# YukunXia/SuperPoint-Stereo-Visual-Odometry

Measured on AMD Instinct MI355X. Metric: stereo frames/sec (1241x376 KITTI), higher is better.
Workload: dtype f32

## Files before the change

### superpoint-stereo-visual-odometry_amd/csrc/conv_wino2.hip.h

```cpp
#pragma once
#include <hip/hip_runtime.h>
#include <stdint.h>
#include <type_traits>
#include <vector>
#include "conv_mfma.hip.h"

#ifndef SPVO_STATIC_BANDS
#define SPVO_STATIC_BANDS 1
#endif

namespace spvo {

#ifndef WINO_STORE_AUX
#define WINO_STORE_AUX 0
#endif

struct WinoTile {
  static constexpr int CK = 8, TH = 8, TW = 32, LW = TW + 8, LH = TH + 2;
  static constexpr int IN_FLOATS = CK * LH * LW;
  static constexpr int U_FLOATS = 16 * CK * CO_TILE;
  static constexpr int W_FLOATS = U_FLOATS + CO_TILE;
  static constexpr int V_FLOATS = 16 * CK * 64;
  static constexpr int RAW_OFF = 0, U_OFF = 2 * IN_FLOATS, V_OFF = U_OFF + 2 * W_FLOATS;
  static constexpr int LDS_BYTES = (V_OFF + 2 * V_FLOATS) * 4;
};

constexpr int WINO2_LDS_BYTES = WinoTile::LDS_BYTES + 16;

inline std::vector<float> pack_conv_weights_wino2(const float *w, const float *bias, int cout, int cin, int cot = CO_TILE) {
  constexpr int CK = WinoTile::CK;
  const int co_tiles = (cout + cot - 1) / cot, nch = cin / CK, ncq = cot / 16;
  const int u_floats = 16 * CK * cot, w_floats = u_floats + cot;
  std::vector<float> out((size_t)co_tiles * nch * w_floats, 0.f);
  static const double G[4][3] = {{1, 0, 0}, {0.5, 0.5, 0.5}, {0.5, -0.5, 0.5}, {0, 0, 1}};
  for (int ct = 0; ct < co_tiles; ++ct)
    for (int ch = 0; ch < nch; ++ch) {
      float *slab = out.data() + ((size_t)ct * nch + ch) * w_floats;
      for (int o = 0; o < cot; ++o) {
        const int co = ct * cot + o;
        if (co >= cout) continue;
        for (int c = 0; c < CK; ++c) {
          const float *g = w + ((size_t)co * cin + ch * CK + c) * 9;
          double t[4][3];
          for (int a = 0; a < 4; ++a)
            for (int k = 0; k < 3; ++k) t[a][k] = G[a][0] * g[0 * 3 + k] + G[a][1] * g[1 * 3 + k] + G[a][2] * g[2 * 3 + k];
          const int lane = 16 * (c & 3) + (o & 15), s = c >> 2, cq = o >> 4;
          for (int a = 0; a < 4; ++a)
            for (int b = 0; b < 4; ++b)
              slab[((((a * 4 + b) >> 1) * ncq + cq) * 64 + lane) * 4 + 2 * ((a * 4 + b) & 1) + s] = (float)(t[a][0] * G[b][0] + t[a][1] * G[b][1] + t[a][2] * G[b][2]);
        }
        if (ch == 0) slab[u_floats + o] = bias[co];
      }
    }
  return out;
}

template <bool POOL, bool RELU, int TAG = 0, bool ODD = false, bool NARROW = false>
__global__ __launch_bounds__(512, 2) void conv_wino2_kernel(const ConvArgs a) {
  using T = WinoTile;
  constexpr int CK = T::CK, LW = T::LW, LH = T::LH, LW4 = LW / 4;
  constexpr int COT = NARROW ? 32 : 64, NCQ = COT / 16, NBLK = NARROW ? 1 : 2;
  constexpr int U_FL = 16 * CK * COT, W_FL = U_FL + COT;
  constexpr int IN_V4 = T::IN_FLOATS / 4, W_V4 = W_FL / 4;
  constexpr int NIT_R = (IN_V4 + 511) / 512, NIT_U = (W_V4 + 511) / 512;
  typedef float f32x2 __attribute__((ext_vector_type(2)));
  typedef float f32x4v __attribute__((ext_vector_type(4)));

  extern __shared__ __attribute__((aligned(16))) float smem[];

  const int tid = threadIdx.x;
  const int lane = tid & 63;
  const int c16 = lane & 15, g4 = lane >> 4;
  const int wave = __builtin_amdgcn_readfirstlane(tid >> 6);
  const int cq = wave % NCQ, tb = wave / NCQ;
  const size_t in_plane = (size_t)a.in_hp * a.in_wp;
  const size_t out_plane = (size_t)a.out_hp * a.out_wp;
  const int n_tiles = a.tiles_x * a.tiles_y * a.co_tiles * a.batch;

  struct TileRef { const float *in_base, *w_base; int x0, y0, ct, img; };
  auto decode = [&](int id) {
    TileRef t;
    const int tx = id % a.tiles_x;
    id /= a.tiles_x;
    const int ty = id % a.tiles_y;
    id /= a.tiles_y;
    t.ct = id % a.co_tiles;
    t.img = id / a.co_tiles;
    t.x0 = tx * T::TW;
    t.y0 = ty * T::TH;
    t.in_base = a.in + ((size_t)t.img * a.in_ctot + a.in_coff) * in_plane + (size_t)(t.y0 + PADY - 1) * a.in_wp + (t.x0 + PADX - 4);
    t.w_base = a.wpack + (size_t)t.ct * a.n_chunks * W_FL;
    return t;
  };

  unsigned roff[NIT_R];
#pragma unroll
  for (int it = 0; it < NIT_R; ++it) {
    const int idx = min(it * 512 + tid, IN_V4 - 1);
    const int ci = idx / (LH * LW4);
    const int rem = idx - ci * (LH * LW4);
    const int r = rem / LW4;
    const int q = rem - r * LW4;
    roff[it] = 4u * (unsigned)(ci * (int)in_plane + r * a.in_wp + q * 4);
  }
  auto issue_raw = [&](const TileRef &t, int chunk, float *buf) {
    const char *inb = reinterpret_cast<const char *>(t.in_base + (size_t)chunk * CK * in_plane);
#pragma unroll
    for (int it = 0; it < NIT_R; ++it)
      if (it < NIT_R - 1 || it * 512 + tid < IN_V4) glds16(reinterpret_cast<const float *>(inb + roff[it]), buf + (it * 512 + wave * 64) * 4);
  };
// ... 106 lines not shown
      if (q.id < n_tiles) q.t = decode(q.id);
    }
  };
  Cursor cu{cur, 0, tile_id};
  issue_raw(cu.t, 0, smem + T::RAW_OFF);
  issue_u(cu.t, 0, smem + T::U_OFF);
  advance(cu);
  if (cu.id < n_tiles) issue_raw(cu.t, cu.chunk, smem + T::RAW_OFF + T::IN_FLOATS);
  Cursor cr = cu;
  advance(cr);
  asm volatile("s_waitcnt vmcnt(0)\n\ts_barrier" ::: "memory");
  transform(smem + T::RAW_OFF, smem + T::V_OFF);

#ifdef WINO_STAMPS
  unsigned long long st_dma = 0, st_bar = 0, st_mfma = 0, st_epi = 0, st_items = 0;
  const unsigned long long st_t0 = __builtin_amdgcn_s_memtime(), st_r0 = __builtin_amdgcn_s_memrealtime();
#endif
  int k = 0;
  bool drained = true;
  constexpr unsigned OOB = 0xFFFFFFFFu;

  while (tile_id < n_tiles) {
    if (a.sched) {
      if (tid == 0) dyn_fetch = band_lo(band) + band_wgs(band) + atomicAdd(a.sched + band, 1);
    } else {
      nxt_id = tile_id + gridDim.x;
    }

    f32x4v acc[16][NBLK];
    auto item = [&](auto first_tag, bool publish) {
      constexpr bool FIRST = decltype(first_tag)::value;
#ifdef WINO_STAMPS
      const unsigned long long ts0 = __builtin_amdgcn_s_memtime();
#endif
      if (!drained) asm volatile("s_waitcnt vmcnt(0)" ::: "memory");
      drained = false;
#ifdef WINO_STAMPS
      const unsigned long long ts1 = __builtin_amdgcn_s_memtime();
#endif
      if (publish && tid == 0) *sched_slot = dyn_fetch < band_hi(band) ? dyn_fetch : n_tiles;
      asm volatile("s_waitcnt lgkmcnt(0)\n\ts_barrier" ::: "memory");
      if (publish) nxt_id = __builtin_amdgcn_readfirstlane(*sched_slot);
#ifdef WINO_STAMPS
      const unsigned long long ts2 = __builtin_amdgcn_s_memtime();
      st_dma += ts1 - ts0; st_bar += ts2 - ts1;
#endif
      const float *ub = smem + T::U_OFF + (k & 1) * T::W_FLOATS;
      const float *vb = smem + T::V_OFF + (k & 1) * T::V_FLOATS;
      float *u_next = smem + T::U_OFF + ((k + 1) & 1) * T::W_FLOATS;
      float *raw_next2 = smem + T::RAW_OFF + (k & 1) * T::IN_FLOATS;
      const float *raw_next = smem + T::RAW_OFF + ((k + 1) & 1) * T::IN_FLOATS;
      float *v_next = smem + T::V_OFF + ((k + 1) & 1) * T::V_FLOATS;
      const f32x4v *vb4 = reinterpret_cast<const f32x4v *>(vb);
      {
        f32x4v avq[2];
        f32x4v bv[4];
        const f32x4v *ub4 = reinterpret_cast<const f32x4v *>(ub);
        auto lda = [&](int g, int p) { avq[p] = ub4[a_lane + (2 * g + p) * (64 * NCQ)]; };
        auto ld = [&](int g, int x) {
          if constexpr (NARROW) {
            const f32x2 b2 = reinterpret_cast<const f32x2 *>(vb)[b_lane + (4 * g + x) * 256];
            bv[x][0] = b2[0]; bv[x][1] = b2[1];
          } else {
            bv[x] = vb4[b_lane + (4 * g + x) * 128];
          }
        };
        lda(0, 0); lda(0, 1);
#pragma unroll
        for (int x = 0; x < 4; ++x) ld(0, x);
#pragma unroll
        for (int g = 0; g < 4; ++g) {
          constexpr int QN = NARROW ? 8 : 16;
#pragma unroll
          for (int q = 0; q < QN; ++q) {
            const int s = NARROW ? q >> 2 : q >> 3, x = NARROW ? q & 3 : (q >> 1) & 3, blk = NARROW ? 0 : q & 1;
            const float a_op = avq[x >> 1][2 * (x & 1) + s];
            if (FIRST && s == 0) acc[4 * g + x][blk] = __builtin_amdgcn_mfma_f32_16x16x4f32(a_op, bv[x][2 * blk + s], f32x4v{0.f, 0.f, 0.f, 0.f}, 0, 0, 0);
            else acc[4 * g + x][blk] = __builtin_amdgcn_mfma_f32_16x16x4f32(a_op, bv[x][2 * blk + s], acc[4 * g + x][blk], 0, 0, 0);
            __builtin_amdgcn_sched_barrier(0);
#ifndef WINO2_ABL
#define WINO2_ABL 0
#endif
#ifndef WINO2_SPREAD
#define WINO2_SPREAD 0
#endif
            const int slot = QN * g + q;
            if (!(WINO2_ABL & 2)) {
              if (WINO2_SPREAD) {
                if (slot >= 1 && slot < 1 + 2 * NIT_U && (slot & 1) && cu.id < n_tiles) issue_u_piece(cu.t, cu.chunk, u_next, (slot - 1) >> 1);
                if (slot >= 1 + 2 * NIT_U && slot < 1 + 2 * NIT_U + 2 * NIT_R && (slot & 1) && cr.id < n_tiles) issue_raw_piece(cr.t, cr.chunk, raw_next2, (slot - 1 - 2 * NIT_U) >> 1);
              } else {
                if (slot == 1 && cu.id < n_tiles) issue_u(cu.t, cu.chunk, u_next);
                if (slot == 5 && cr.id < n_tiles) issue_raw(cr.t, cr.chunk, raw_next2);
              }
            }
            if (!(WINO2_ABL & 4) && g < 3 && q >= QN - 4) {
              ld(g + 1, q - (QN - 4));
              if (q == QN - 4 + (NARROW ? 1 : 0)) lda(g + 1, 0);
              if (q == QN - 1) lda(g + 1, 1);
            }
            if constexpr (NARROW) {
              if (!(WINO2_ABL & 1) && slot >= 8 && slot < 28) xf_step(raw_next, v_next, slot - 8);
            } else {
              if (!(WINO2_ABL & 1) && slot >= 16 && slot < 56 && !(slot & 1)) xf_step(raw_next, v_next, (slot - 16) >> 1);
            }
            __builtin_amdgcn_sched_barrier(0);
          }
        }
      }
      if (FIRST) {
        const float bias_a = g4 ? 0.f : ub[U_FL + cq * 16 + c16];
#pragma unroll
        for (int blk = 0; blk < NBLK; ++blk) acc[5][blk] = __builtin_amdgcn_mfma_f32_16x16x4f32(bias_a, 1.0f, acc[5][blk], 0, 0, 0);
      }
      advance(cu);
      advance(cr);
      ++k;
#ifdef WINO_STAMPS
      st_mfma += __builtin_amdgcn_s_memtime() - ts2;
      ++st_items;
#endif
    };
    item(std::true_type{}, false);
    for (int c = 1; c < a.n_chunks; ++c) item(std::false_type{}, a.sched != nullptr && c == 1);

    asm volatile("s_waitcnt vmcnt(0)" ::: "memory");
    drained = true;

#ifdef WINO_STAMPS
    const unsigned long long te0 = __builtin_amdgcn_s_memtime();
#endif
    float *co_base = a.out + (((size_t)cur.img * a.out_ctot + a.out_coff) + (size_t)cur.ct * COT + cq * 16) * out_plane;
    const __amdgpu_buffer_rsrc_t rsrc = __builtin_amdgcn_make_buffer_rsrc(co_base, 0, 0x7FFFFFFF, 0x00020000);
    const int oplane = (int)out_plane;
    const int kmax = a.cout - (cur.ct * COT + cq * 16 + 4 * g4);
    auto relu = [](float v) { return RELU ? __builtin_amdgcn_fmed3f(v, 0.f, __builtin_inff()) : v; };
#pragma unroll
    for (int blk = 0; blk < NBLK; ++blk) {
// ... 60 lines not shown
```

### superpoint-stereo-visual-odometry_amd/csrc/spvo_core.hip

```cpp
#include "spvo_internal.hip.h"
#include <mutex>
#include "conv_mfma.hip.h"
#include "conv_f16.hip.h"
#include "conv_bf16x3.hip.h"
#include "conv_wino2.hip.h"
#include "conv_wino4.hip.h"
#include "heads.hip.h"
#include "conv_i8.hip.h"
#include "conv_i8_fused.hip.h"
#include "heads_i8.hip.h"

namespace spvo_int {

thread_local std::string g_error;
HostDiag g_diag;

int fail(spvo_ctx *c, int code, const char *fmt, ...) {
  char buf[512];
  va_list ap;
  va_start(ap, fmt);
  vsnprintf(buf, sizeof buf, fmt, ap);
  va_end(ap);
  if (c) c->error = buf;
  g_error = buf;
  return code;
}

int stage_id(spvo_ctx *c, const std::string &name) {
  for (size_t i = 0; i < c->stages.size(); ++i)
    if (c->stages[i].name == name) return (int)i;
  Stage s;
  s.name = name;
  c->stages.push_back(s);
  return (int)c->stages.size() - 1;
}

namespace {
const char *const kTuningNames[] = {"winograd", "wino4", "wino4_item", "wino_narrow", "wino_dynamic", "winograd_min_tiles", "wino4_min_tiles", "merge_siblings", "heads_fused",
                                    "heads_on_net", "heads_split", "match_fused", "fp32_split", "prematch", "spin_wait", "trunk_timing", "solve_timing", "nms_first", "upload_side", "inject_launch_failure", "int8_fused", "pair_always", "preprocess_fused", "heads_keep_raw", "tail_streams", "solve_collect_first", "graphs", "solve_fuse", "solve_keep", "sift_describe_form", "sift_pair_waves_per_cu", "conv_variant"};
constexpr int kTuningCount = sizeof kTuningNames / sizeof kTuningNames[0];
std::mutex g_tuning_mutex;
bool g_tuning_set[kTuningCount] = {};
int g_tuning_value[kTuningCount] = {};
int tuning_index(const char *name) {
  for (int i = 0; name && i < kTuningCount; ++i)
    if (std::strcmp(name, kTuningNames[i]) == 0) return i;
  return -1;
}
}
int tuning(const char *name, int dflt) {
  const int i = tuning_index(name);
  if (i < 0) return dflt;
  std::lock_guard<std::mutex> lock(g_tuning_mutex);
  return g_tuning_set[i] ? g_tuning_value[i] : dflt;
}

bool spin_wait_enabled() { return tuning("spin_wait", 0) != 0; }
hipError_t wait_event(hipEvent_t ev) {
  if (spin_wait_enabled()) {
    for (long spins = 0; spins < 20000000; ++spins) {
      const hipError_t e = hipEventQuery(ev);
      if (e != hipErrorNotReady) return e;
      __builtin_ia32_pause();
    }
  }
  return hipEventSynchronize(ev);
}

hipEvent_t get_event(spvo_ctx *c) {
  if (!c->free_events.empty()) {
    hipEvent_t e = c->free_events.back();
    c->free_events.pop_back();
    return e;
  }
  hipEvent_t e;
  (void)hipEventCreate(&e);
  return e;
}

void resolve_pending(spvo_ctx *c) {
  if (c->pending.empty()) return;
  for (auto &p : c->pending) {
    float ms = 0;
    (void)hipEventSynchronize(p.e1);
    if (hipEventElapsedTime(&ms, p.e0, p.e1) == hipSuccess) {
      c->stages[p.stage].total_ms += ms;
      c->stages[p.stage].calls += 1;
      c->stages[p.stage].flops_sum += p.flops;
      c->stages[p.stage].bytes_sum += p.bytes;
    }
    c->free_events.push_back(p.e0);
// ... 694 lines not shown
          HIP_TRY(c, hipMemcpy(op.d_b, b, (size_t)op.cout * 4, hipMemcpyHostToDevice));
          continue;
        }
        const int ckg = op.ks == 3 ? 1 : 2;
        if (op.cin % (8 * ckg) || op.in_c_off % 8) return fail(c, SPVO_ERR_IO, "op %u: cin %d / channel offset %d do not fit the split-fp32 chunking (%d)", i, op.cin, op.in_c_off, 8 * ckg);
        op.ck = 8 * ckg;
        op.n_chunks = op.cin / op.ck;
        op.co_tiles = (op.cout + CO_TILE - 1) / CO_TILE;
        int ck_unused;
        choose_variant(op.ks, ti.H, ti.W, op.co_tiles, c->cfg.max_batch, pool, c->num_cus, &op.wr, &op.wc, &ck_unused, true);
        const std::vector<unsigned short> pk = pack_conv_weights_s3(w, b, op.cout, op.cin, op.ks, ckg);
        int rc = dev_alloc(c, &op.d_ws3, pk.size(), false);
        if (rc) return rc;
        HIP_TRY(c, hipMemcpy(op.d_ws3, pk.data(), pk.size() * sizeof(unsigned short), hipMemcpyHostToDevice));
        continue;
      }
      if (op.cin == 1) {
        if (pool || add) return fail(c, SPVO_ERR_IO, "op %u: single-channel-input layers have no pooling / residual form", i);
        int rc = dev_alloc(c, &op.d_w, (size_t)op.cout * taps, false);
        if (rc) return rc;
        if ((rc = dev_alloc(c, &op.d_b, op.cout, false))) return rc;
        HIP_TRY(c, hipMemcpy(op.d_w, w, (size_t)op.cout * taps * 4, hipMemcpyHostToDevice));
        HIP_TRY(c, hipMemcpy(op.d_b, b, (size_t)op.cout * 4, hipMemcpyHostToDevice));
        continue;
      }
      op.co_tiles = (op.cout + CO_TILE - 1) / CO_TILE;
      choose_variant(op.ks, ti.H, ti.W, op.co_tiles, c->cfg.max_batch, pool, c->num_cus, &op.wr, &op.wc, &op.ck);
      {
        const bool wino_on = tuning("winograd", 1) != 0;
        const long wtiles = (long)((ti.W + WinoTile::TW - 1) / WinoTile::TW) * ((ti.H + WinoTile::TH - 1) / WinoTile::TH) * op.co_tiles * c->cfg.max_batch;
        const long min_tiles = tuning("winograd_min_tiles", 3 * c->num_cus / 4);
        const bool eligible = wino_on && op.ks == 3 && !bn && !add && (op.cin % WinoTile::CK) == 0 && (!pool || ((ti.H % 2) == 0 && (ti.W % 2) == 0));
        op.wino = eligible && wtiles >= min_tiles;
        if (eligible && !op.wino && tuning("wino_narrow", 1) && (op.cout % 32) == 0 && 3 * wtiles >= min_tiles) op.wino = op.wino_narrow = true;
      }
      const bool dynamic_tiles = tuning("wino_dynamic", 1) != 0;
      if (op.wino && !op.wino_narrow && (op.cin % Wino4Tile::CK) == 0 && (((ti.H | ti.W) & 1) == 0 || !pool) && tuning("wino4", 1)) {
        const long t4 = (long)((ti.W + Wino4Tile::TW - 1) / Wino4Tile::TW) * ((ti.H + Wino4Tile::TH - 1) / Wino4Tile::TH) * op.co_tiles * c->cfg.max_batch;
        if (t4 >= tuning("wino4_min_tiles", 3 * c->num_cus / 4)) {
          op.wino4 = true;
          op.wino4_item = tuning("wino4_item", 1) != 0;
          op.ck = Wino4Tile::CK;
          op.n_chunks = op.cin / Wino4Tile::CK;
          const std::vector<float> pk = pack_conv_weights_wino4(w, b, op.cout, op.cin);
          int rc = dev_alloc(c, &op.d_w, pk.size(), false);
          if (rc) return rc;
          HIP_TRY(c, hipMemcpy(op.d_w, pk.data(), pk.size() * 4, hipMemcpyHostToDevice));
          if (dynamic_tiles && (rc = dev_alloc(c, &op.d_sched, 16))) return rc;
          continue;
        }
      }
      if (op.wino) {
        op.ck = WinoTile::CK;
        op.n_chunks = op.cin / op.ck;
        if (op.wino_narrow) op.co_tiles = op.cout / 32;
        const std::vector<float> pk = pack_conv_weights_wino2(w, b, op.cout, op.cin, op.wino_narrow ? 32 : CO_TILE);
        int rc = dev_alloc(c, &op.d_w, pk.size(), false);
        if (rc) return rc;
        HIP_TRY(c, hipMemcpy(op.d_w, pk.data(), pk.size() * 4, hipMemcpyHostToDevice));
        if (dynamic_tiles && (rc = dev_alloc(c, &op.d_sched, 16))) return rc;
        continue;
      }
      if (op.cin % op.ck) return fail(c, SPVO_ERR_IO, "op %u: cin %d is not a multiple of %d", i, op.cin, op.ck);
      op.n_chunks = op.cin / op.ck;
      const std::vector<float> pk = pack_conv_weights(w, b, op.cout, op.cin, op.ks, op.ck);
      std::vector<float> bp((size_t)op.co_tiles * CO_TILE, 0.f);
      for (int o = 0; o < op.cout; ++o) bp[o] = b[o];
      int rc = dev_alloc(c, &op.d_w, pk.size(), false);
      if (rc) return rc;
      if ((rc = dev_alloc(c, &op.d_b, bp.size(), false))) return rc;
      HIP_TRY(c, hipMemcpy(op.d_w, pk.data(), pk.size() * 4, hipMemcpyHostToDevice));
      HIP_TRY(c, hipMemcpy(op.d_b, bp.data(), bp.size() * 4, hipMemcpyHostToDevice));
    } else if (op.type == OP_MAXPOOL) {
      std::snprintf(name, sizeof name, "pool:%u", i);
      op.stage = stage_id(c, name);
      if (to.level != ti.level + 1 || to.ch != ti.ch) return fail(c, SPVO_ERR_IO, "op %u: bad pool", i);
    } else if (op.type == OP_L2NORM) {
      std::snprintf(name, sizeof name, "l2norm:%u", i);
      op.stage = stage_id(c, name);
      if (ti.ch != 256 || to.ch != 256 || ti.level != 3) return fail(c, SPVO_ERR_IO, "op %u: descriptor tail must be 256 channels at 1/8", i);
    } else {
      return fail(c, SPVO_ERR_IO, "op %u: unknown type %d", i, op.type);
    }
  }
  if (!c->int8 && !c->s3 && c->head_start + 3 == c->ops.size() && tuning("heads_fused", 1)) {
    const size_t hs = c->head_start;
    const Op &pb = c->ops[hs], &db = c->ops[hs + 1], &nm = c->ops[hs + 2];
    const bool plain = pb.type == OP_CONV && db.type == OP_CONV && nm.type == OP_L2NORM && pb.ks == 1 && db.ks == 1 && pb.flags == 0 && db.flags == 0 &&
                       pb.cin == HEADS_CIN && db.cin == HEADS_CIN && pb.cout == 65 && db.cout == 256 && pb.out == c->t_det && pb.out_c_off == 0 &&
                       db.out_c_off == 0 && nm.in == db.out && nm.out == c->t_desc && c->tensors[pb.in].level == 3 && c->tensors[db.in].level == 3 &&
                       !c->tensors[pb.in].nhwc && !c->tensors[db.in].nhwc && !pb.merged && !db.merged &&
                       c->tensors[pb.in].f16 == c->fp16 && c->tensors[db.in].f16 == c->fp16 && (!c->fp16 || ((pb.in_c_off | db.in_c_off) % 8) == 0);
    if (plain) {
      const std::vector<float> pk = pack_heads_weights(payload + raws[hs].w_off, payload + raws[hs].b_off, pb.cout, payload + raws[hs + 1].w_off, payload + raws[hs + 1].b_off, c->fp16);
      int rc = dev_alloc(c, &c->d_heads_w, pk.size(), false);
      if (rc) return rc;
      HIP_TRY(c, hipMemcpy(c->d_heads_w, pk.data(), pk.size() * 4, hipMemcpyHostToDevice));
      c->heads_fused = true;
    }
  }
  if (c->int8 && c->head_start + 3 == c->ops.size() && tuning("heads_fused", 1)) {
    const size_t hs = c->head_start;
    const Op &pb = c->ops[hs], &db = c->ops[hs + 1], &nm = c->ops[hs + 2];
    const bool plain = pb.type == OP_CONV && db.type == OP_CONV && nm.type == OP_L2NORM && pb.ks == 1 && db.ks == 1 && pb.flags == 0 && db.flags == 0 &&
                       pb.cin == HEADS8_CIN && db.cin == HEADS8_CIN && pb.cout == 65 && db.cout == 256 && pb.out == c->t_det && pb.out_c_off == 0 &&
                       db.out_c_off == 0 && nm.in == db.out && nm.out == c->t_desc && c->tensors[pb.in].level == 3 && c->tensors[db.in].level == 3 &&
// ... 169 lines not shown
```

### superpoint-stereo-visual-odometry_amd/csrc/spvo_internal.hip.h

```cpp
#pragma once
#include <hip/hip_runtime.h>

#include <algorithm>
#include <cmath>
#include <cstdarg>
#include <cstdio>
#include <cstdlib>
#include <cstring>
#include <string>
#include <vector>
#include <deque>
#include <time.h>

#include "../../include/spvo.h"
#include "spvo_types.hip.h"

#pragma GCC visibility push(hidden)
namespace spvo { struct BriskLongPair; struct BriskShortPair; }
using namespace spvo;

#include "launch_segments.hip.h"

namespace spvo_int {

constexpr int RING = 8;
constexpr int MAX_INFLIGHT = 6;
constexpr int N_SLOTS = 16;
constexpr int N_BIN_SLOTS = 10;
constexpr int N_SIFT_SLOTS = 10;
constexpr int SIFT_SLOT_MAX = 32768;
constexpr int BIN_COUNTER_INTS = 16;
constexpr int HAM_KEY_SHIFT = 22;

struct Tensor {
  int ch = 0, level = 0, H = 0, W = 0, hp = 0, wp = 0;
  bool nhwc = false;
  bool f16 = false;
  bool i8 = false;
  bool s3 = false;
  float scale = 0.f;
  float *d = nullptr;
  float *dr[RING] = {};
  size_t per_image = 0;
};

enum { OP_CONV = 1, OP_MAXPOOL = 2, OP_L2NORM = 3, OP_DWCONV = 4 };
enum { FLAG_RELU = 1, FLAG_POOL = 2, FLAG_BN = 4, FLAG_ADD = 8 };

struct Op {
  int type = 0, in = 0, out = 0, out_c_off = 0, in_c_off = 0, cin = 0, cout = 0, ks = 0, flags = 0;
  int ck = 0, n_chunks = 0, co_tiles = 0, wr = 0, wc = 0;
  int residual = 0;
  bool merged = false;
  bool wino = false;
  bool wino_narrow = false;
  bool wino4 = false;
  bool wino4_item = true;
  bool dominant = false;
  float *d_w = nullptr, *d_b = nullptr, *d_bn_scale = nullptr, *d_bn_shift = nullptr;
  int *d_sched = nullptr;
  _Float16 *d_w16 = nullptr;
  int8_t *d_w8 = nullptr;
  unsigned short *d_ws3 = nullptr;
  int *d_wq32 = nullptr;
  int *d_wsel = nullptr;
  int fused_dw = -1;
  bool fused_stem = false;
  bool fused_away = false;
  float *d_qm = nullptr;
  float inv_s_out = 0.f, s_res = 0.f;
  double flops_per_image = 0;
  int stage = -1;
  mutable int launch_tiles = 0, launch_wgs = 0;
};

struct Stage {
  std::string name;
  double total_ms = 0;
  long long calls = 0;
  double flops = 0, bytes = 0;
  double flops_sum = 0, bytes_sum = 0;
};

struct Pending { int stage; hipEvent_t e0, e1; double flops = 0, bytes = 0; };

struct SlotState {
  int n = 0;
  bool filled = false;
  int *d_n = nullptr;
  unsigned long long gen = 0;
};
inline void slot_rewrite(SlotState &s) { s.filled = false; s.n = 0; ++s.gen; }

struct FeatureSlot : SlotState {
  int *d_xy = nullptr;
  float *d_desc = nullptr;
  float *d_sqn = nullptr;
};

struct BinarySlot : SlotState {
  OrbKeypoint *d_kp = nullptr;
  uint32_t *d_desc = nullptr;
  int row_bytes = 32;
};

struct SiftSlot : SlotState {
  float *d_desc = nullptr;
  float *d_sqn = nullptr;
  SiftSrc *d_src = nullptr;
};
// ... 537 lines not shown
```

### superpoint-stereo-visual-odometry_amd/csrc/spvo_net_f32.hip

```cpp
#include "spvo_internal.hip.h"
#include "conv_mfma.hip.h"
#include "conv_wino2.hip.h"
#include "conv_wino4.hip.h"
#include "heads.hip.h"

namespace spvo_int {

template <int KS, int CK, int WR, int WC, bool POOL, bool RELU, int EPI = 0, int MINW = 1, int TAG = 0>
int launch_conv_instance(spvo_ctx *c, ConvArgs args, hipStream_t stream) {
  using T = ConvTile<KS, CK, WR, WC>;
  auto k = conv_mfma_kernel<KS, CK, WR, WC, POOL, RELU, MINW, 0, EPI, TAG>;
  static int per_cu[64] = {};
  const int dev = c->cfg.device & 63;
  if (!per_cu[dev]) {
    HIP_TRY(c, hipFuncSetAttribute((const void *)k, hipFuncAttributeMaxDynamicSharedMemorySize, T::LDS_BYTES));
    int n = 0;
    HIP_TRY(c, hipOccupancyMaxActiveBlocksPerMultiprocessor(&n, (const void *)k, 256, T::LDS_BYTES));
    per_cu[dev] = std::max(n, 1);
  }
  const int n_tiles = args.tiles_x * args.tiles_y * args.co_tiles * args.batch;
  const int grid = std::min(n_tiles, c->num_cus * per_cu[dev]);
  c->launch_tiles = n_tiles; c->launch_wgs = grid;
  hipLaunchKernelGGL(k, dim3(grid), dim3(256), T::LDS_BYTES, stream, args);
  HIP_TRY(c, hipGetLastError());
  return SPVO_OK;
}

template <int KS, int CK, int WR, int WC, bool POOL, int MINW = 1>
int launch_conv_variant(spvo_ctx *c, const ConvArgs &a, int batch, bool relu, hipStream_t stream, bool dominant = false) {
  using T = ConvTile<KS, CK, WR, WC>;
  ConvArgs args = a;
  args.tiles_x = (a.W + T::TW - 1) / T::TW;
  args.tiles_y = (a.H + T::TH - 1) / T::TH;
  args.batch = batch;
  if constexpr (KS == 3) {
    if (dominant && relu) return launch_conv_instance<KS, CK, WR, WC, POOL, true, 0, MINW, 1>(c, args, stream);
  }
  return relu ? launch_conv_instance<KS, CK, WR, WC, POOL, true, 0, MINW>(c, args, stream)
              : launch_conv_instance<KS, CK, WR, WC, POOL, false, 0, MINW>(c, args, stream);
}

template <int WR, int WC, bool POOL>
int launch_conv_epi(spvo_ctx *c, const ConvArgs &a, int batch, int epi, hipStream_t stream) {
  using T = ConvTile<1, 16, WR, WC>;
  ConvArgs args = a;
  args.tiles_x = (a.W + T::TW - 1) / T::TW;
  args.tiles_y = (a.H + T::TH - 1) / T::TH;
  args.batch = batch;
  return epi == 1 ? launch_conv_instance<1, 16, WR, WC, POOL, true, 1>(c, args, stream)
                  : launch_conv_instance<1, 16, WR, WC, POOL, false, 2>(c, args, stream);
}

template <bool POOL, bool RELU, int TAG, bool ODD = false, bool NARROW = false>
int launch_conv_wino_instance(spvo_ctx *c, const ConvArgs &args, hipStream_t stream) {
  static bool ready[64] = {};
  const int dev = c->cfg.device & 63;
  const int n_tiles = args.tiles_x * args.tiles_y * args.co_tiles * args.batch;
  const int rounds = (n_tiles + c->num_cus - 1) / c->num_cus;
  const int grid = (n_tiles + rounds - 1) / rounds;
  auto k = conv_wino2_kernel<POOL, RELU, TAG, ODD, NARROW>;
  if (!ready[dev]) {
    HIP_TRY(c, hipFuncSetAttribute((const void *)k, hipFuncAttributeMaxDynamicSharedMemorySize, WINO2_LDS_BYTES));
    ready[dev] = true;
  }
  ConvArgs a2 = args;
  if (rounds < 2 || args.n_chunks < 4) a2.sched = nullptr;
  hipLaunchKernelGGL(k, dim3(grid), dim3(512), WINO2_LDS_BYTES, stream, a2);
  HIP_TRY(c, hipGetLastError());
  return SPVO_OK;
}

int launch_conv_wino_sel(spvo_ctx *c, const ConvArgs &args, bool relu, bool pool, bool dominant, bool narrow, hipStream_t stream) {
  const ConvArgs &a = args;
  if (narrow) {
    if (!pool && ((a.H | a.W) & 1)) return relu ? launch_conv_wino_instance<false, true, 0, true, true>(c, args, stream) : launch_conv_wino_instance<false, false, 0, true, true>(c, args, stream);
    if (pool) return relu ? launch_conv_wino_instance<true, true, 0, false, true>(c, args, stream) : launch_conv_wino_instance<true, false, 0, false, true>(c, args, stream);
    return relu ? launch_conv_wino_instance<false, true, 0, false, true>(c, args, stream) : launch_conv_wino_instance<false, false, 0, false, true>(c, args, stream);
  }
  if (!pool && ((a.H | a.W) & 1)) return relu ? launch_conv_wino_instance<false, true, 0, true>(c, args, stream) : launch_conv_wino_instance<false, false, 0, true>(c, args, stream);
  if (dominant && relu) return pool ? launch_conv_wino_instance<true, true, 1, false>(c, args, stream) : launch_conv_wino_instance<false, true, 1, false>(c, args, stream);
  if (pool) return relu ? launch_conv_wino_instance<true, true, 0, false>(c, args, stream) : launch_conv_wino_instance<true, false, 0, false>(c, args, stream);
  return relu ? launch_conv_wino_instance<false, true, 0, false>(c, args, stream) : launch_conv_wino_instance<false, false, 0, false>(c, args, stream);
}

template <bool POOL, bool RELU, int TAG, bool ITEM>
int launch_conv_wino4_instance(spvo_ctx *c, const ConvArgs &args, hipStream_t stream) {
  static bool ready[64] = {};
  const int dev = c->cfg.device & 63;
  auto k = conv_wino4_kernel<POOL, RELU, TAG, 2, ITEM>;
  if (!ready[dev]) {
    HIP_TRY(c, hipFuncSetAttribute((const void *)k, hipFuncAttributeMaxDynamicSharedMemorySize, Wino4Tile::LDS_BYTES));
    ready[dev] = true;
  }
  const int n_tiles = args.tiles_x * args.tiles_y * args.co_tiles * args.batch;
  const int rounds = (n_tiles + c->num_cus - 1) / c->num_cus;
  const int grid = (n_tiles + rounds - 1) / rounds;
  ConvArgs a2 = args;
  if (rounds < 2 || args.n_chunks < 5) a2.sched = nullptr;
  hipLaunchKernelGGL(k, dim3(grid), dim3(512), Wino4Tile::LDS_BYTES, stream, a2);
  HIP_TRY(c, hipGetLastError());
  return SPVO_OK;
}

template <bool ITEM>
int launch_conv_wino4_sel(spvo_ctx *c, const ConvArgs &args, bool relu, bool pool, bool dominant, hipStream_t stream) {
  if (dominant && relu) return pool ? launch_conv_wino4_instance<true, true, 1, ITEM>(c, args, stream) : launch_conv_wino4_instance<false, true, 1, ITEM>(c, args, stream);
  if (pool) return relu ? launch_conv_wino4_instance<true, true, 0, ITEM>(c, args, stream) : launch_conv_wino4_instance<true, false, 0, ITEM>(c, args, stream);
  return relu ? launch_conv_wino4_instance<false, true, 0, ITEM>(c, args, stream) : launch_conv_wino4_instance<false, false, 0, ITEM>(c, args, stream);
}

int launch_conv_wino4(spvo_ctx *c, const ConvArgs &a, int batch, bool relu, bool pool, bool dominant, bool new_item, hipStream_t stream) {
  ConvArgs args = a;
  args.tiles_x = (a.W + Wino4Tile::TW - 1) / Wino4Tile::TW;
  args.tiles_y = (a.H + Wino4Tile::TH - 1) / Wino4Tile::TH;
  args.batch = batch;
  if (pool && ((a.H | a.W) & 1)) return fail(c, SPVO_ERR_INVALID, "F(4x4) kernel: pooled layer with odd size");
  return new_item ? launch_conv_wino4_sel<true>(c, args, relu, pool, dominant, stream) : launch_conv_wino4_sel<false>(c, args, relu, pool, dominant, stream);
}

int launch_conv_wino(spvo_ctx *c, const ConvArgs &a, int batch, bool relu, bool pool, bool dominant, bool narrow, hipStream_t stream) {
  ConvArgs args = a;
  args.tiles_x = (a.W + WinoTile::TW - 1) / WinoTile::TW;
  args.tiles_y = (a.H + WinoTile::TH - 1) / WinoTile::TH;
  args.batch = batch;
  return launch_conv_wino_sel(c, args, relu, pool, dominant, narrow, stream);
}

int launch_conv(spvo_ctx *c, const Op &op, int img0, int batch, hipStream_t stream) {
  const Tensor &ti = c->tensors[op.in];
  const Tensor &to = c->tensors[op.out];
  const float *tin = ring_ptr(c, ti, img0);
  float *tout = ring_ptr(c, to, img0);
  const bool relu = op.flags & FLAG_RELU, pool = op.flags & FLAG_POOL;
  const int epi = (op.flags & FLAG_BN) ? 1 : (op.flags & FLAG_ADD) ? 2 : 0;
  if (op.type == OP_DWCONV) {
    dim3 grid((ti.W + 255) / 256, (ti.H + 3) / 4, batch * op.cout);
    if (relu)
      hipLaunchKernelGGL(dwconv3x3_kernel<true>, grid, dim3(256), 0, stream, tin, tout, op.d_w, op.d_b, op.cout, ti.H, ti.W, ti.hp, ti.wp);
    else
      hipLaunchKernelGGL(dwconv3x3_kernel<false>, grid, dim3(256), 0, stream, tin, tout, op.d_w, op.d_b, op.cout, ti.H, ti.W, ti.hp, ti.wp);
    HIP_TRY(c, hipGetLastError());
    return SPVO_OK;
  }
  if (op.cin == 1) {
    dim3 grid((ti.W + 63) / 64, (ti.H + 3) / 4, batch);
#define SPVO_FIRST(KS, RELU) hipLaunchKernelGGL((conv_first_kernel<KS, RELU>), grid, dim3(256), 0, stream, tin, tout, op.d_w, op.d_b, \
                                                op.d_bn_scale, op.d_bn_shift, ti.H, ti.W, ti.hp, ti.wp, to.ch, op.out_c_off, op.cout, 0)
    if (op.ks == 3 && !op.d_bn_scale) {
      dim3 g4((ti.W + 255) / 256, (ti.H + 3) / 4, batch);
      if (relu) hipLaunchKernelGGL(conv_first4_kernel<true>, g4, dim3(256), 0, stream, tin, tout, op.d_w, op.d_b, ti.H, ti.W, ti.hp, ti.wp, to.ch, op.out_c_off, op.cout);
      else hipLaunchKernelGGL(conv_first4_kernel<false>, g4, dim3(256), 0, stream, tin, tout, op.d_w, op.d_b, ti.H, ti.W, ti.hp, ti.wp, to.ch, op.out_c_off, op.cout);
    } else if (op.ks == 3) { if (relu) SPVO_FIRST(3, true); else SPVO_FIRST(3, false); }
    else            { if (relu) SPVO_FIRST(1, true); else SPVO_FIRST(1, false); }
#undef SPVO_FIRST
    HIP_TRY(c, hipGetLastError());
    return SPVO_OK;
  }
  ConvArgs a;
  a.in = tin; a.out = tout; a.wpack = op.d_w; a.bias = op.d_b;
  a.H = ti.H; a.W = ti.W;
  a.in_hp = ti.hp; a.in_wp = ti.wp; a.in_ctot = ti.ch; a.in_coff = op.in_c_off;
  a.out_hp = to.hp; a.out_wp = to.wp; a.out_ctot = to.ch; a.out_coff = op.out_c_off;
  a.cout = op.cout; a.n_chunks = op.n_chunks; a.co_tiles = op.co_tiles;
  a.tiles_x = a.tiles_y = 0;
  a.batch = batch;
  a.sched = op.d_sched;
  if (op.wino4) return launch_conv_wino4(c, a, batch, relu, pool, op.dominant, op.wino4_item, stream);
  if (op.wino) return launch_conv_wino(c, a, batch, relu, pool, op.dominant, op.wino_narrow, stream);
  const int key = op.ks * 10000 + op.ck * 100 + op.wr * 20 + op.wc * 2 + (pool ? 1 : 0);
  if (epi) {
    a.bn_scale = op.d_bn_scale; a.bn_shift = op.d_bn_shift;
    if (epi == 2) a.residual = ring_ptr(c, c->tensors[op.residual], img0);
    switch (key) {
      case 11644: return launch_conv_epi<2, 2, false>(c, a, batch, epi, stream);
      case 11624: return launch_conv_epi<1, 2, false>(c, a, batch, epi, stream);
      case 11622: return launch_conv_epi<1, 1, false>(c, a, batch, epi, stream);
      case 11645: return launch_conv_epi<2, 2, true>(c, a, batch, epi, stream);
      case 11643: return launch_conv_epi<2, 1, true>(c, a, batch, epi, stream);
      default: return fail(c, SPVO_ERR_INVALID, "no conv kernel variant for key %d with epilogue %d", key, epi);
    }
  }
  switch (key) {
    case 30844: return launch_conv_variant<3, 8, 2, 2, false, 1>(c, a, batch, relu, stream, op.dominant);
    case 30842: return launch_conv_variant<3, 8, 2, 1, false, 2>(c, a, batch, relu, stream, op.dominant);
    case 30824: return launch_conv_variant<3, 8, 1, 2, false, 2>(c, a, batch, relu, stream, op.dominant);
    case 30822: return launch_conv_variant<3, 8, 1, 1, false, 4>(c, a, batch, relu, stream, op.dominant);
    case 30845: return launch_conv_variant<3, 8, 2, 2, true, 1>(c, a, batch, relu, stream, op.dominant);
    case 30843: return launch_conv_variant<3, 8, 2, 1, true, 2>(c, a, batch, relu, stream, op.dominant);
    case 11644: return launch_conv_variant<1, 16, 2, 2, false>(c, a, batch, relu, stream);
    case 11624: return launch_conv_variant<1, 16, 1, 2, false>(c, a, batch, relu, stream);
    case 11622: return launch_conv_variant<1, 16, 1, 1, false>(c, a, batch, relu, stream);
    case 11645: return launch_conv_variant<1, 16, 2, 2, true>(c, a, batch, relu, stream);
    case 11643: return launch_conv_variant<1, 16, 2, 1, true>(c, a, batch, relu, stream);
    default: return fail(c, SPVO_ERR_INVALID, "no conv kernel variant for key %d", key);
  }
}

int launch_op(spvo_ctx *c, const Op &op, int img0, int batch, hipStream_t stream) {
  if (op.merged || op.fused_away) return SPVO_OK;
  const Tensor &ti = c->tensors[op.in];
  const Tensor &to = c->tensors[op.out];
  if (op.type == OP_CONV || op.type == OP_DWCONV) {
    auto esz = [](const Tensor &t) { return t.i8 ? 1.0 : (t.f16 || t.s3) ? (t.s3 ? 6.0 : 2.0) : 4.0; };
    const double wsz = c->int8 ? 1.0 : (c->fp16 ? 2.0 : (c->s3 ? 6.0 : 4.0));
    const double bytes = batch * ((double)op.cin * ti.H * ti.W * esz(ti) + (double)op.cout * to.H * to.W * esz(to)) +
                         (double)op.cout * (op.type == OP_DWCONV ? 1 : op.cin) * op.ks * op.ks * wsz;
    if (op.fused_dw >= 0) {
      const Op &dw = c->ops[op.fused_dw];
      const Tensor &t0 = c->tensors[op.fused_stem ? c->ops[0].in : dw.in];
      double fl = op.flops_per_image + dw.flops_per_image, by = (double)t0.ch * t0.H * t0.W * esz(t0) + (double)op.cout * to.H * to.W * esz(to);
      if (op.fused_stem) fl += c->ops[0].flops_per_image + c->ops[1].flops_per_image;
      ScopedStage st(c, op.stage, fl * batch, batch * by + (double)op.cout * op.cin + 9.0 * dw.cout, stream);
      return launch_conv8(c, op, img0, batch, stream);
    }
    ScopedStage st(c, op.stage, op.flops_per_image * batch, bytes, stream);
    c->launch_tiles = c->launch_wgs = 0;
    const int rc = c->int8 ? launch_conv8(c, op, img0, batch, stream) : c->fp16 ? launch_conv16(c, op, img0, batch, stream)
                   : c->s3 ? launch_conv_s3(c, op, img0, batch, stream) : launch_conv(c, op, img0, batch, stream);
    op.launch_tiles = c->launch_tiles; op.launch_wgs = c->launch_wgs;
    return rc;
  }
// ... 74 lines not shown
```

Measured before the change: 1552.

## Software-pipeline wino2 MFMA loop with explicit LDS reads and lgkmcnt waits

Adds an ITEM variant of the Winograd F(2,3) kernel's inner MFMA loop. Operand loads are issued as inline-asm ds_read instructions a fixed number of slots ahead (LEAD), and each MFMA waits on lgkmcnt counts computed at compile time, so only the reads it needs must have landed. The input transform's LDS reads and writes are folded into the same slot schedule. This aims to hide LDS latency behind MFMAs better than the old per-group prefetch, at the cost of more live registers and fragile hand-computed wait counts. A tuning flag selects the new path and defaults to on.

```diff
diff --git a/superpoint-stereo-visual-odometry_amd/csrc/conv_wino2.hip.h b/superpoint-stereo-visual-odometry_amd/csrc/conv_wino2.hip.h
--- a/superpoint-stereo-visual-odometry_amd/csrc/conv_wino2.hip.h
+++ b/superpoint-stereo-visual-odometry_amd/csrc/conv_wino2.hip.h
@@ -2,6 +2,7 @@
 #include <hip/hip_runtime.h>
 #include <stdint.h>
 #include <type_traits>
+#include <utility>
 #include <vector>
 #include "conv_mfma.hip.h"
 
@@ -55,7 +56,65 @@
   return out;
 }
 
-template <bool POOL, bool RELU, int TAG = 0, bool ODD = false, bool NARROW = false>
+#ifndef WINO2_ABL
+#define WINO2_ABL 0
+#endif
+#ifndef WINO2_SPREAD
+#define WINO2_SPREAD 0
+#endif
+#ifndef WINO2_ITEM_LEAD_NARROW
+#define WINO2_ITEM_LEAD_NARROW 4
+#endif
+#ifndef WINO2_ITEM_LEAD_WIDE
+#define WINO2_ITEM_LEAD_WIDE 16
+#endif
+
+constexpr int wino2_nm(bool narrow) { return narrow ? 32 : 64; }
+constexpr int wino2_qn(bool narrow) { return wino2_nm(narrow) / 4; }
+constexpr int wino2_s(int p, bool narrow) { return narrow ? (p % 8) >> 2 : (p % 16) >> 3; }
+constexpr int wino2_x(int p, bool narrow) { return narrow ? p & 3 : (p >> 1) & 3; }
+constexpr int wino2_blk(int p, bool narrow) { return narrow ? 0 : p & 1; }
+constexpr int wino2_a_piece(int p, bool narrow) { return 2 * (p / wino2_qn(narrow)) + (wino2_x(p, narrow) >> 1); }
+constexpr int wino2_b_piece(int p, bool narrow) { return 4 * (p / wino2_qn(narrow)) + wino2_x(p, narrow); }
+constexpr int wino2_first_slot_a(int j, bool narrow) { return wino2_qn(narrow) * (j / 2) + (narrow ? 2 : 4) * (j & 1); }
+constexpr int wino2_first_slot_b(int j, bool narrow) { return wino2_qn(narrow) * (j / 4) + (narrow ? 1 : 2) * (j & 3); }
+constexpr bool wino2_slot_reads_a(int q, bool narrow) { return q < wino2_nm(narrow) && wino2_first_slot_a(wino2_a_piece(q, narrow), narrow) == q; }
+constexpr bool wino2_slot_reads_b(int q, bool narrow) { return q < wino2_nm(narrow) && wino2_first_slot_b(wino2_b_piece(q, narrow), narrow) == q; }
+constexpr int wino2_reads_before(int q_end, bool narrow) {
+  int n = 0;
+  for (int q = 0; q < q_end && q < wino2_nm(narrow); ++q) n += (wino2_slot_reads_a(q, narrow) ? 1 : 0) + (wino2_slot_reads_b(q, narrow) ? 1 : 0);
+  return n;
+}
+constexpr int wino2_xf_step_at(int slot, bool narrow) {
+  if (narrow) return slot >= 8 && slot < 28 ? slot - 8 : -1;
+  return slot >= 16 && slot < 56 && !(slot & 1) ? (slot - 16) >> 1 : -1;
+}
+constexpr int wino2_xf_slot(int st, bool narrow) { return narrow ? 8 + st : 16 + 2 * st; }
+constexpr int wino2_xf_ops(int st) { return st < 0 ? 0 : st < 12 ? 1 : st < 16 ? 0 : 2; }
+constexpr int wino2_slot_reads(int q, bool narrow) { return (wino2_slot_reads_a(q, narrow) ? 1 : 0) + (wino2_slot_reads_b(q, narrow) ? 1 : 0); }
+constexpr int wino2_issued_before(int p, int lead, bool narrow, bool xf) {
+  int n = wino2_reads_before(lead, narrow);
+  for (int i = 0; i < p; ++i) n += wino2_slot_reads(i + lead, narrow) + (xf ? wino2_xf_ops(wino2_xf_step_at(i, narrow)) : 0);
+  return n;
+}
+constexpr int wino2_read_index(int q, bool second, int lead, bool narrow, bool xf) {
+  return (q < lead ? wino2_reads_before(q, narrow) : wino2_issued_before(q - lead, lead, narrow, xf)) + (second ? 1 : 0);
+}
+constexpr int wino2_wait_count(int p, int lead, bool narrow, bool xf) {
+  const int qa = wino2_first_slot_a(wino2_a_piece(p, narrow), narrow), qb = wino2_first_slot_b(wino2_b_piece(p, narrow), narrow);
+  const int ia = wino2_read_index(qa, false, lead, narrow, xf), ib = wino2_read_index(qb, wino2_slot_reads_a(qb, narrow), lead, narrow, xf);
+  const int n = wino2_issued_before(p, lead, narrow, xf) - 1 - (ia > ib ? ia : ib);
+  return n < 0 ? 0 : (n > 15 ? 15 : n);
+}
+constexpr int wino2_xf_wait_count(int st, int j, int lead, bool narrow) {
+  const int ps = wino2_xf_slot(st, narrow), pj = wino2_xf_slot(j, narrow);
+  const int n = wino2_issued_before(ps, lead, narrow, true) + wino2_slot_reads(ps + lead, narrow) - 1 - (wino2_issued_before(pj, lead, narrow, true) + wino2_slot_reads(pj + lead, narrow));
+  return n < 0 ? 0 : (n > 15 ? 15 : n);
+}
+template <class F, int... P>
+__device__ __forceinline__ void wino2_for_each(F &&f, std::integer_sequence<int, P...>) { (f(std::integral_constant<int, P>{}), ...); }
+
+template <bool POOL, bool RELU, int TAG = 0, bool ODD = false, bool NARROW = false, bool ITEM = true>
 __global__ __launch_bounds__(512, 2) void conv_wino2_kernel(const ConvArgs a) {
   using T = WinoTile;
   constexpr int CK = T::CK, LW = T::LW, LH = T::LH, LW4 = LW / 4;
@@ -268,7 +327,71 @@
       const float *raw_next = smem + T::RAW_OFF + ((k + 1) & 1) * T::IN_FLOATS;
       float *v_next = smem + T::V_OFF + ((k + 1) & 1) * T::V_FLOATS;
       const f32x4v *vb4 = reinterpret_cast<const f32x4v *>(vb);
-      {
+      if constexpr (ITEM) {
+        constexpr int LEAD = NARROW ? WINO2_ITEM_LEAD_NARROW : WINO2_ITEM_LEAD_WIDE, NM = wino2_nm(NARROW);
+        constexpr bool XF = !(WINO2_ABL & 1);
+        static_assert(LEAD >= 1 && LEAD <= NM, "WINO2_ITEM_LEAD");
+        static_assert(!WINO2_SPREAD && !(WINO2_ABL & 4), "these experiments exist in the ITEM = 0 form only");
+        f32x4v av[8];
+        f32x4v bw[16];
+        f32x2 bn[16];
+        const unsigned ua = (unsigned)(uintptr_t)(const __attribute__((address_space(3))) void *)(reinterpret_cast<const f32x4v *>(ub) + a_lane);
+        const unsigned va = NARROW ? (unsigned)(uintptr_t)(const __attribute__((address_space(3))) void *)(reinterpret_cast<const f32x2 *>(vb) + b_lane)
+                                   : (unsigned)(uintptr_t)(const __attribute__((address_space(3))) void *)(vb4 + b_lane);
+        const unsigned ra = (unsigned)(uintptr_t)(const __attribute__((address_space(3))) void *)(raw_next + raw_off - 1);
+        const unsigned wa = (unsigned)(uintptr_t)(const __attribute__((address_space(3))) void *)(v_next + v_off);
+        auto read_slot = [&av, &bw, &bn, ua, va](auto qc) __attribute__((always_inline)) {
+          constexpr int q = decltype(qc)::value;
+          if constexpr (wino2_slot_reads_a(q, NARROW)) {
+            constexpr int j = wino2_a_piece(q, NARROW);
+            asm volatile("ds_read_b128 %0, %1 offset:%2" : "=v"(av[j]) : "v"(ua), "n"(j * 64 * NCQ * 16));
+          }
+          if constexpr (wino2_slot_reads_b(q, NARROW)) {
+            constexpr int j = wino2_b_piece(q, NARROW);
+            if constexpr (NARROW) asm volatile("ds_read_b64 %0, %1 offset:%2" : "=v"(bn[j]) : "v"(va), "n"(j * 256 * 8));
+            else asm volatile("ds_read_b128 %0, %1 offset:%2" : "=v"(bw[j]) : "v"(va), "n"(j * 128 * 16));
+          }
+        };
+        auto step = [&](auto pc) __attribute__((always_inline)) {
+          constexpr int p = decltype(pc)::value;
+          constexpr int s = wino2_s(p, NARROW), x = wino2_x(p, NARROW), blk = wino2_blk(p, NARROW), pos = 4 * (p / wino2_qn(NARROW)) + x;
+          constexpr int ja = wino2_a_piece(p, NARROW), jb = wino2_b_piece(p, NARROW);
+          if constexpr (wino2_slot_reads_a(p, NARROW) || wino2_slot_reads_b(p, NARROW)) {
+            if constexpr (NARROW) asm volatile("s_waitcnt lgkmcnt(%2)" : "+v"(av[ja]), "+v"(bn[jb]) : "n"(wino2_wait_count(p, LEAD, NARROW, XF)));
+            else asm volatile("s_waitcnt lgkmcnt(%2)" : "+v"(av[ja]), "+v"(bw[jb]) : "n"(wino2_wait_count(p, LEAD, NARROW, XF)));
+          }
+          const float a_op = av[ja][2 * (x & 1) + s];
+          float b_op;
+          if constexpr (NARROW) b_op = bn[jb][s];
+          else b_op = bw[jb][2 * blk + s];
+          if (FIRST && s == 0) acc[pos][blk] = __builtin_amdgcn_mfma_f32_16x16x4f32(a_op, b_op, f32x4v{0.f, 0.f, 0.f, 0.f}, 0, 0, 0);
+          else acc[pos][blk] = __builtin_amdgcn_mfma_f32_16x16x4f32(a_op, b_op, acc[pos][blk], 0, 0, 0);
+          __builtin_amdgcn_sched_barrier(0);
+          if (!(WINO2_ABL & 2) && p == 1 && cu.id < n_tiles) issue_u(cu.t, cu.chunk, u_next);
+          if (!(WINO2_ABL & 2) && p == 5 && cr.id < n_tiles) issue_raw(cr.t, cr.chunk, raw_next2);
+          read_slot(std::integral_constant<int, p + LEAD>{});
+          constexpr int st = wino2_xf_step_at(p, NARROW);
+          if constexpr (XF && st >= 0) {
+            if constexpr (st < 12) {
+              asm volatile("ds_read_b64 %0, %1 offset:%2" : "=v"(dp[st]) : "v"(ra), "n"(((st / 3) * LW + 2 * (st % 3)) * 4));
+            } else if constexpr (st < 16) {
+              if constexpr (st != 14) {
+                constexpr int c = st == 12 ? 0 : st == 13 ? 1 : 2;
+                asm volatile("s_waitcnt lgkmcnt(%4)" : "+v"(dp[c]), "+v"(dp[3 + c]), "+v"(dp[6 + c]), "+v"(dp[9 + c]) : "n"(wino2_xf_wait_count(st, 9 + c, LEAD, NARROW)));
+              }
+              xf_step(raw_next, v_next, st);
+            } else {
+              constexpr int r = st - 16;
+              const float o0 = tt[r * 4 + 0] - tt[r * 4 + 2], o1 = tt[r * 4 + 1] + tt[r * 4 + 2], o2 = tt[r * 4 + 2] - tt[r * 4 + 1], o3 = tt[r * 4 + 1] - tt[r * 4 + 3];
+              asm volatile("ds_write2st64_b32 %0, %1, %2 offset0:%3 offset1:%4" : : "v"(wa), "v"(o0), "v"(o1), "n"((4 * r + 0) * 8), "n"((4 * r + 1) * 8));
+              asm volatile("ds_write2st64_b32 %0, %1, %2 offset0:%3 offset1:%4" : : "v"(wa), "v"(o2), "v"(o3), "n"((4 * r + 2) * 8), "n"((4 * r + 3) * 8));
+            }
+          }
+          __builtin_amdgcn_sched_barrier(0);
+        };
+        wino2_for_each(read_slot, std::make_integer_sequence<int, LEAD>{});
+        wino2_for_each(step, std::make_integer_sequence<int, NM>{});
+      } else {
         f32x4v avq[2];
         f32x4v bv[4];
         const f32x4v *ub4 = reinterpret_cast<const f32x4v *>(ub);
@@ -294,12 +417,6 @@
             if (FIRST && s == 0) acc[4 * g + x][blk] = __builtin_amdgcn_mfma_f32_16x16x4f32(a_op, bv[x][2 * blk + s], f32x4v{0.f, 0.f, 0.f, 0.f}, 0, 0, 0);
             else acc[4 * g + x][blk] = __builtin_amdgcn_mfma_f32_16x16x4f32(a_op, bv[x][2 * blk + s], acc[4 * g + x][blk], 0, 0, 0);
             __builtin_amdgcn_sched_barrier(0);
-#ifndef WINO2_ABL
-#define WINO2_ABL 0
-#endif
-#ifndef WINO2_SPREAD
-#define WINO2_SPREAD 0
-#endif
             const int slot = QN * g + q;
             if (!(WINO2_ABL & 2)) {
               if (WINO2_SPREAD) {
diff --git a/superpoint-stereo-visual-odometry_amd/csrc/spvo_core.hip b/superpoint-stereo-visual-odometry_amd/csrc/spvo_core.hip
--- a/superpoint-stereo-visual-odometry_amd/csrc/spvo_core.hip
+++ b/superpoint-stereo-visual-odometry_amd/csrc/spvo_core.hip
@@ -36,7 +36,7 @@
 }
 
 namespace {
-const char *const kTuningNames[] = {"winograd", "wino4", "wino4_item", "wino_narrow", "wino_dynamic", "winograd_min_tiles", "wino4_min_tiles", "merge_siblings", "heads_fused",
+const char *const kTuningNames[] = {"winograd", "wino4", "wino4_item", "wino2_item", "wino_narrow", "wino_dynamic", "winograd_min_tiles", "wino4_min_tiles", "merge_siblings", "heads_fused",
                                     "heads_on_net", "heads_split", "match_fused", "fp32_split", "prematch", "spin_wait", "trunk_timing", "solve_timing", "nms_first", "upload_side", "inject_launch_failure", "int8_fused", "pair_always", "preprocess_fused", "heads_keep_raw", "tail_streams", "solve_collect_first", "graphs", "solve_fuse", "solve_keep", "sift_describe_form", "sift_pair_waves_per_cu", "conv_variant"};
 constexpr int kTuningCount = sizeof kTuningNames / sizeof kTuningNames[0];
 std::mutex g_tuning_mutex;
@@ -837,6 +837,7 @@
       }
       if (op.wino) {
         op.ck = WinoTile::CK;
+        op.wino2_item = tuning("wino2_item", 1) != 0;
         op.n_chunks = op.cin / op.ck;
         if (op.wino_narrow) op.co_tiles = op.cout / 32;
         const std::vector<float> pk = pack_conv_weights_wino2(w, b, op.cout, op.cin, op.wino_narrow ? 32 : CO_TILE);
diff --git a/superpoint-stereo-visual-odometry_amd/csrc/spvo_internal.hip.h b/superpoint-stereo-visual-odometry_amd/csrc/spvo_internal.hip.h
--- a/superpoint-stereo-visual-odometry_amd/csrc/spvo_internal.hip.h
+++ b/superpoint-stereo-visual-odometry_amd/csrc/spvo_internal.hip.h
@@ -56,6 +56,7 @@
   bool wino_narrow = false;
   bool wino4 = false;
   bool wino4_item = true;
+  bool wino2_item = true;
   bool dominant = false;
   float *d_w = nullptr, *d_b = nullptr, *d_bn_scale = nullptr, *d_bn_shift = nullptr;
   int *d_sched = nullptr;
diff --git a/superpoint-stereo-visual-odometry_amd/csrc/spvo_net_f32.hip b/superpoint-stereo-visual-odometry_amd/csrc/spvo_net_f32.hip
--- a/superpoint-stereo-visual-odometry_amd/csrc/spvo_net_f32.hip
+++ b/superpoint-stereo-visual-odometry_amd/csrc/spvo_net_f32.hip
@@ -51,14 +51,14 @@
                   : launch_conv_instance<1, 16, WR, WC, POOL, false, 2>(c, args, stream);
 }
 
-template <bool POOL, bool RELU, int TAG, bool ODD = false, bool NARROW = false>
+template <bool ITEM, bool POOL, bool RELU, int TAG, bool ODD = false, bool NARROW = false>
 int launch_conv_wino_instance(spvo_ctx *c, const ConvArgs &args, hipStream_t stream) {
   static bool ready[64] = {};
   const int dev = c->cfg.device & 63;
   const int n_tiles = args.tiles_x * args.tiles_y * args.co_tiles * args.batch;
   const int rounds = (n_tiles + c->num_cus - 1) / c->num_cus;
   const int grid = (n_tiles + rounds - 1) / rounds;
-  auto k = conv_wino2_kernel<POOL, RELU, TAG, ODD, NARROW>;
+  auto k = conv_wino2_kernel<POOL, RELU, TAG, ODD, NARROW, ITEM>;
   if (!ready[dev]) {
     HIP_TRY(c, hipFuncSetAttribute((const void *)k, hipFuncAttributeMaxDynamicSharedMemorySize, WINO2_LDS_BYTES));
     ready[dev] = true;
@@ -70,17 +70,18 @@
   return SPVO_OK;
 }
 
+template <bool ITEM>
 int launch_conv_wino_sel(spvo_ctx *c, const ConvArgs &args, bool relu, bool pool, bool dominant, bool narrow, hipStream_t stream) {
   const ConvArgs &a = args;
   if (narrow) {
-    if (!pool && ((a.H | a.W) & 1)) return relu ? launch_conv_wino_instance<false, true, 0, true, true>(c, args, stream) : launch_conv_wino_instance<false, false, 0, true, true>(c, args, stream);
-    if (pool) return relu ? launch_conv_wino_instance<true, true, 0, false, true>(c, args, stream) : launch_conv_wino_instance<true, false, 0, false, true>(c, args, stream);
-    return relu ? launch_conv_wino_instance<false, true, 0, false, true>(c, args, stream) : launch_conv_wino_instance<false, false, 0, false, true>(c, args, stream);
-  }
-  if (!pool && ((a.H | a.W) & 1)) return relu ? launch_conv_wino_instance<false, true, 0, true>(c, args, stream) : launch_conv_wino_instance<false, false, 0, true>(c, args, stream);
-  if (dominant && relu) return pool ? launch_conv_wino_instance<true, true, 1, false>(c, args, stream) : launch_conv_wino_instance<false, true, 1, false>(c, args, stream);
-  if (pool) return relu ? launch_conv_wino_instance<true, true, 0, false>(c, args, stream) : launch_conv_wino_instance<true, false, 0, false>(c, args, stream);
-  return relu ? launch_conv_wino_instance<false, true, 0, false>(c, args, stream) : launch_conv_wino_instance<false, false, 0, false>(c, args, stream);
+    if (!pool && ((a.H | a.W) & 1)) return relu ? launch_conv_wino_instance<ITEM, false, true, 0, true, true>(c, args, stream) : launch_conv_wino_instance<ITEM, false, false, 0, true, true>(c, args, stream);
+    if (pool) return relu ? launch_conv_wino_instance<ITEM, true, true, 0, false, true>(c, args, stream) : launch_conv_wino_instance<ITEM, true, false, 0, false, true>(c, args, stream);
+    return relu ? launch_conv_wino_instance<ITEM, false, true, 0, false, true>(c, args, stream) : launch_conv_wino_instance<ITEM, false, false, 0, false, true>(c, args, stream);
+  }
+  if (!pool && ((a.H | a.W) & 1)) return relu ? launch_conv_wino_instance<ITEM, false, true, 0, true>(c, args, stream) : launch_conv_wino_instance<ITEM, false, false, 0, true>(c, args, stream);
+  if (dominant && relu) return pool ? launch_conv_wino_instance<ITEM, true, true, 1, false>(c, args, stream) : launch_conv_wino_instance<ITEM, false, true, 1, false>(c, args, stream);
+  if (pool) return relu ? launch_conv_wino_instance<ITEM, true, true, 0, false>(c, args, stream) : launch_conv_wino_instance<ITEM, true, false, 0, false>(c, args, stream);
+  return relu ? launch_conv_wino_instance<ITEM, false, true, 0, false>(c, args, stream) : launch_conv_wino_instance<ITEM, false, false, 0, false>(c, args, stream);
 }
 
 template <bool POOL, bool RELU, int TAG, bool ITEM>
@@ -118,12 +119,12 @@
   return new_item ? launch_conv_wino4_sel<true>(c, args, relu, pool, dominant, stream) : launch_conv_wino4_sel<false>(c, args, relu, pool, dominant, stream);
 }
 
-int launch_conv_wino(spvo_ctx *c, const ConvArgs &a, int batch, bool relu, bool pool, bool dominant, bool narrow, hipStream_t stream) {
+int launch_conv_wino(spvo_ctx *c, const ConvArgs &a, int batch, bool relu, bool pool, bool dominant, bool narrow, bool new_item, hipStream_t stream) {
   ConvArgs args = a;
   args.tiles_x = (a.W + WinoTile::TW - 1) / WinoTile::TW;
   args.tiles_y = (a.H + WinoTile::TH - 1) / WinoTile::TH;
   args.batch = batch;
-  return launch_conv_wino_sel(c, args, relu, pool, dominant, narrow, stream);
+  return new_item ? launch_conv_wino_sel<true>(c, args, relu, pool, dominant, narrow, stream) : launch_conv_wino_sel<false>(c, args, relu, pool, dominant, narrow, stream);
 }
 
 int launch_conv(spvo_ctx *c, const Op &op, int img0, int batch, hipStream_t stream) {
@@ -166,7 +167,7 @@
   a.batch = batch;
   a.sched = op.d_sched;
   if (op.wino4) return launch_conv_wino4(c, a, batch, relu, pool, op.dominant, op.wino4_item, stream);
-  if (op.wino) return launch_conv_wino(c, a, batch, relu, pool, op.dominant, op.wino_narrow, stream);
+  if (op.wino) return launch_conv_wino(c, a, batch, relu, pool, op.dominant, op.wino_narrow, op.wino2_item, stream);
   const int key = op.ks * 10000 + op.ck * 100 + op.wr * 20 + op.wc * 2 + (pool ? 1 : 0);
   if (epi) {
     a.bn_scale = op.d_bn_scale; a.bn_shift = op.d_bn_shift;
```

Result: no change. 1553 (median of 4 runs) (+0.1%).
